# davidfang00/opticalflowdiffusion

Hardware: AMD Instinct MI355X
Metric: UNet denoise steps/sec @ 2x436x1024 flow, bs=16 (higher is better)
Workload: dtype bf16

## Files before the change

opticalflowdiffusion_amd/csrc/conv_common.h:

```cpp
#pragma once
#include "common.h"
#include "conv_params.h"
#include "mfma_util.h"

namespace ofd {

__device__ __forceinline__ float silu_f(float y) { return y * __builtin_amdgcn_rcpf(1.0f + __expf(-y)); }

static inline bool plain_epilogue(const ConvParams& P) {
    return !P.residual && !P.residual_b && !P.res_act && !P.split && !P.pool2 && !P.out2;
}

__device__ __forceinline__ u32x4 prologue_octet(u32x4 v, const float (&ps)[8], const float (&pb)[8]) {
#pragma unroll
    for (int j = 0; j < 4; ++j) {
        const float lo = silu_f(bf2f((bf16_t)(v[j] & 0xffffu)) * ps[2 * j] + pb[2 * j]);
        const float hi = silu_f(bf2f((bf16_t)(v[j] >> 16)) * ps[2 * j + 1] + pb[2 * j + 1]);
        v[j] = f2bf2(lo, hi);
    }
    return v;
}

__device__ __forceinline__ void load_in_affine8(const ConvParams& P, int b, int c_chunk, int c_oct, float (&ps)[8], float (&pb)[8]) {
    const float* sp = P.in_scale + (size_t)b * P.Cin_total + c_chunk + c_oct;
    const float* bp = P.in_shift + (size_t)b * P.Cin_total + c_chunk + c_oct;
    *(float4*)&ps[0] = *(const float4*)sp; *(float4*)&ps[4] = *(const float4*)(sp + 4);
    *(float4*)&pb[0] = *(const float4*)bp; *(float4*)&pb[4] = *(const float4*)(bp + 4);
}

__device__ __forceinline__ void split_quads(const uint4 t4, uint2& lo, uint2& hi) {
    const auto sx = __builtin_amdgcn_permlane32_swap(t4.x, t4.z, false, false);
    const auto sy = __builtin_amdgcn_permlane32_swap(t4.y, t4.w, false, false);
    lo = make_uint2(sx[0], sy[0]);
    hi = make_uint2(sx[1], sy[1]);
}

__device__ __forceinline__ void add_residual4(float (&v)[4], const uint2 t) {
    v[0] += bf2f((bf16_t)(t.x & 0xffffu));
    v[1] += bf2f((bf16_t)(t.x >> 16));
    v[2] += bf2f((bf16_t)(t.y & 0xffffu));
    v[3] += bf2f((bf16_t)(t.y >> 16));
}
__device__ __forceinline__ void add_silu_affine4(float (&v)[4], const uint2 t, const float4 sc, const float4 sh) {
    v[0] += silu_f(bf2f((bf16_t)(t.x & 0xffffu)) * sc.x + sh.x);
    v[1] += silu_f(bf2f((bf16_t)(t.x >> 16)) * sc.y + sh.y);
    v[2] += silu_f(bf2f((bf16_t)(t.y & 0xffffu)) * sc.z + sh.z);
    v[3] += silu_f(bf2f((bf16_t)(t.y >> 16)) * sc.w + sh.w);
}

__device__ __forceinline__ void gn_stat_add(const uint2 q, float& sum, float& sumsq) {
    typedef __bf16 bf16x2 __attribute__((ext_vector_type(2)));
    const bf16x2 one = __builtin_bit_cast(bf16x2, 0x3f803f80u);
    const bf16x2 va = __builtin_bit_cast(bf16x2, q.x), vb = __builtin_bit_cast(bf16x2, q.y);
    sum = __builtin_amdgcn_fdot2_f32_bf16(vb, one, __builtin_amdgcn_fdot2_f32_bf16(va, one, sum, false), false);
    sumsq = __builtin_amdgcn_fdot2_f32_bf16(vb, vb, __builtin_amdgcn_fdot2_f32_bf16(va, va, sumsq, false), false);
}

namespace wp {

constexpr int CK = 32, NC = CK / 8, IW = 34, TW = 32, RING = 6, FRAGS = 18;

template <int NS, int PH>
struct Cfg {
    static constexpr int NTHREADS = 64 * NS * PH;
    static constexpr int BN = 32 * NS, ROWS = 8 * PH, IH = ROWS + 2, NPIX = IH * IW;
    static constexpr int NC = wp::NC;
    static constexpr int US = (NPIX + 1) * 16;
    static constexpr int XB = NC * US;
    static constexpr int LDS_BYTES = 2 * XB;
    static constexpr int XPT = (NPIX * NC + NTHREADS - 1) / NTHREADS;
    static_assert(NS * PH == 4, "4 waves");
    static_assert((NPIX + 1) % 2 == 1, "odd slot count keeps the staging writes of a pixel's octets on distinct banks");
};

typedef u32x4 u4;

__device__ __forceinline__ bf16x8 as_frag(u4 v) { return __builtin_bit_cast(bf16x8, v); }

__device__ __forceinline__ void wave_reduce8(float (&v)[8]) {
    const int lane = threadIdx.x & 63;
#pragma unroll
    for (int i = 0; i < 4; ++i) {
        const auto r = __builtin_amdgcn_permlane32_swap(__float_as_uint(v[i]), __float_as_uint(v[i + 4]), false, false);
        v[i] = __uint_as_float(r[0]) + __uint_as_float(r[1]);
    }
#pragma unroll
    for (int i = 0; i < 2; ++i) {
        const auto r = __builtin_amdgcn_permlane16_swap(__float_as_uint(v[i]), __float_as_uint(v[i + 2]), false, false);
        v[i] = __uint_as_float(r[0]) + __uint_as_float(r[1]);
    }
    {
        const bool up = (lane & 8) != 0;
        const float send = up ? v[0] : v[1], keep = up ? v[1] : v[0];
        v[0] = keep + __uint_as_float(__builtin_amdgcn_mov_dpp(__float_as_uint(send), 0x128 , 0xf, 0xf, false));
    }
    v[0] += __uint_as_float(__builtin_amdgcn_mov_dpp(__float_as_uint(v[0]), 0x141 , 0xf, 0xf, false));
    v[0] += __uint_as_float(__builtin_amdgcn_mov_dpp(__float_as_uint(v[0]), 0xb1 , 0xf, 0xf, false));
    v[0] += __uint_as_float(__builtin_amdgcn_mov_dpp(__float_as_uint(v[0]), 0x4e , 0xf, 0xf, false));
}

template <int NS, int OCT>
__device__ __forceinline__ void gn_partial_store_wave(const ConvParams& P, float (&stat)[8], int b, int ty8, int tiles8, int tx, int ns, int oct0, int lane) {
    wave_reduce8(stat);
    if (ty8 < tiles8) {
        constexpr int PER_WAVE = (4 / NS) * OCT * 2;
        const int slot_i = lane / (OCT * 2), o = (lane % (OCT * 2)) >> 1, which = lane & 1;
        const float total = __shfl(stat[0], ((o & 3) * 2 + which) * 8, 64);
        if (lane < PER_WAVE) {
            const int slot = ns + slot_i * NS;
            const bool own = slot_i == 0 && (o >> 2) == ns;
            P.gn_partial[gn_partial_index(b, tiles8 * P.tiles_x * 4, (ty8 * P.tiles_x + tx) * 4 + slot, P.Cout / 8, oct0 + o) + which] = own ? total : 0.0f;
        }
    }
}

template <int BN>
__device__ __forceinline__ bool cy_fast_decode(const ConvParams& P, int ntiles, int& tile, int& cy) {
    tile = blockIdx.x;
    cy = blockIdx.y;
    if (P.cy_fast) {
        const int ny = P.Cout / BN, j = blockIdx.x, g = j >> 3;
        cy = g % ny;
        tile = (g / ny) * 8 + (j & 7);
        if (tile >= ntiles) return false;
    }
    return true;
}

template <class C>
__device__ __forceinline__ void stage_map(const ConvParams& P, int tid, int oy0, int ox0, int (&pyx)[C::XPT], unsigned& okmask) {
    okmask = 0;
#pragma unroll
    for (int i = 0; i < C::XPT; ++i) {
        const int p = min(tid / C::NC + i * (C::NTHREADS / C::NC), C::NPIX - 1);
        const int ty = p / IW, tx = p - ty * IW;
        const int iy = oy0 - 1 + ty, ix = ox0 - 1 + tx;
        const bool ok = iy >= 0 && iy < P.H && ix >= 0 && ix < P.W;
        okmask |= (ok ? 1u : 0u) << i;
        pyx[i] = (min(max(iy, 0), P.H - 1) << 16) | min(max(ix, 0), P.W - 1);
    }
}

template <class C, bool PRO>
__device__ __forceinline__ void stage_write(const u4 (&xs)[C::XPT], unsigned okmask, const float (&ps)[8], const float (&pb)[8], unsigned char* xbuf, int t) {
    const int c8 = t % C::NC;
#pragma unroll
    for (int i = 0; i < C::XPT; ++i) {
        const int p = min(t / C::NC + i * (C::NTHREADS / C::NC), C::NPIX - 1);
        u4 v = xs[i];
        if constexpr (PRO) v = prologue_octet(v, ps, pb);
        const bool ok = (okmask >> i) & 1u;
#pragma unroll
        for (int j = 0; j < 4; ++j) v[j] = ok ? v[j] : 0u;
        *(u4*)(xbuf + c8 * C::US + p * 16) = v;
    }
}

template <class C>
__device__ __forceinline__ void stage_write(const u4 (&xs)[C::XPT], unsigned okmask, unsigned char* xbuf, int t) {
    const float none[8] = {};
    stage_write<C, false>(xs, okmask, none, none, xbuf, t);
}

struct ChunkSrc {
    const bf16_t* base;
    int SW, stride;
    int up;
};
__device__ __forceinline__ ChunkSrc chunk_src(const ConvParams& P, int b, int kc, int c8, int& src_i, int& src_first) {
    const int k64 = kc >> 1;
    while (k64 >= src_first + P.src[src_i].chunks) {
        src_first += P.src[src_i].chunks;
        ++src_i;
    }
    const ConvSrcDev& S = P.src[src_i];
    return {S.ptr + (size_t)b * S.SH * S.SW * S.src_channels + S.ch_offset + (k64 - src_first) * 64 + (kc & 1) * CK + c8 * 8, S.SW, S.src_channels,
            S.mode == 1 ? 1 : 0};
}

template <class C>
__device__ __forceinline__ void load_chunk(const ConvParams& P, int b, int kc, int tid, const int (&pyx)[C::XPT], int& src_i, int& src_first, u4 (&xs)[C::XPT]) {
    const ChunkSrc S = chunk_src(P, b, kc, tid % C::NC, src_i, src_first);
#pragma unroll
    for (int i = 0; i < C::XPT; ++i) {
        const int sy = (pyx[i] >> 16) >> S.up, sx = (pyx[i] & 0xffff) >> S.up;
        xs[i] = *(const u4*)(S.base + ((size_t)sy * S.SW + sx) * S.stride);
    }
}
template <class C, bool PRO>
__device__ __forceinline__ void write_chunk(const ConvParams& P, int b, int kc, int tid, unsigned okmask, const u4 (&xs)[C::XPT], unsigned char* xbuf) {
    float ps[8], pb[8];
    if constexpr (PRO) load_in_affine8(P, b, kc * CK, (tid % C::NC) * 8, ps, pb);
    stage_write<C, PRO>(xs, okmask, ps, pb, xbuf, tid);
}

}

}
```

opticalflowdiffusion_amd/csrc/conv_pc.hip:

```cpp
#include <cstdlib>
#include <type_traits>
#include "conv_common.h"

namespace ofd {

namespace wp {

struct PcCfg {
    using C = Cfg<2, 2>;
    static constexpr int NPROD = C::NTHREADS, XPT = C::XPT;
    static constexpr int WSLOT = FRAGS * 2 * 1024;
    static constexpr int MAX_ITEMS = 512;
    static constexpr int ITEMS_OFF = 2 * C::XB + 2 * WSLOT;
    static constexpr int LDS_BYTES = ITEMS_OFF + MAX_ITEMS * 16;
};

template <bool PRO>
__global__ void __launch_bounds__(512, 2) conv3x3_pc_kernel(const ConvParams P) {
    using C = PcCfg::C;
    constexpr int NPROD = PcCfg::NPROD, XPT = PcCfg::XPT;
    extern __shared__ __attribute__((aligned(16))) unsigned char smem[];
    unsigned char* const wlds = smem + 2 * C::XB;
    const int tid = threadIdx.x;

    const int tiles_y = (P.H + C::ROWS - 1) / C::ROWS;
    const int tpi = P.tiles_x * tiles_y, ntiles = tpi * P.B, ny = P.Cout / C::BN, G = gridDim.x;
    const int nitems = (ntiles + 7) / 8 * 8 * ny;
    const int n32 = P.total_chunks * 2;
    auto decode = [&](int j, int& b, int& oy0, int& ox0, int& cy) -> bool {
        if (j >= nitems) return false;
        const int g = j >> 3;
        cy = ny > 1 ? g % ny : 0;
        int tile = (ny > 1 ? g / ny : g) * 8 + (j & 7);
        if (tile >= ntiles) return false;
        tile = xcd_tile_order(tile, ntiles);
        b = tile / tpi;
        const int t_in = tile - b * tpi;
        oy0 = (t_in / P.tiles_x) * C::ROWS;
        ox0 = (t_in % P.tiles_x) * TW;
        return true;
    };
    const int nit = blockIdx.x < nitems ? min((nitems - 1 - (int)blockIdx.x) / G + 1, PcCfg::MAX_ITEMS) : 0;
    int4* const items = (int4*)(smem + PcCfg::ITEMS_OFF);
    for (int k = tid; k < nit; k += 512) {
        int b_, y_, x_, c_;
        const bool ok = decode(blockIdx.x + k * G, b_, y_, x_, c_);
        items[k] = make_int4(ok ? b_ : -1, y_, x_, c_);
    }
    __syncthreads();
    int nvalid_items = 0;
    if (nit > 0) {
        int lo = 0, hi = nit;
        while (lo < hi) { const int mid = (lo + hi) >> 1; if (items[mid].x >= 0) lo = mid + 1; else hi = mid; }
        nvalid_items = lo;
    }
    const int T = n32 * nvalid_items;
    if (T == 0) return;
    auto item_at = [&](int k, int& b, int& oy0, int& ox0, int& cy) -> bool {
        if (k >= nvalid_items) return false;
        const int4 d = items[k];
        b = __builtin_amdgcn_readfirstlane(d.x); oy0 = __builtin_amdgcn_readfirstlane(d.y);
        ox0 = __builtin_amdgcn_readfirstlane(d.z); cy = __builtin_amdgcn_readfirstlane(d.w);
        return true;
    };

    if (tid >= 256) {
        const int ptid = tid - 256;
        const int c8 = ptid % NC;
        int tyx[XPT];
#pragma unroll
        for (int i = 0; i < XPT; ++i) {
            const int p = min(ptid / NC + i * (NPROD / NC), C::NPIX - 1);
            const int ty = p / IW;
            tyx[i] = (ty << 8) | (p - ty * IW);
        }
        int lk = 0, lkc = 0, lb, loy0, lox0, lcy;
        item_at(0, lb, loy0, lox0, lcy);
        auto advance = [&]() {
            if (++lkc == n32) {
                if (item_at(lk + 1, lb, loy0, lox0, lcy)) { lkc = 0; ++lk; }
                else lkc = n32 - 1;
            }
        };
        auto issue = [&](u4 (&xs)[XPT], unsigned& okmask, float (&ps)[8], float (&pb)[8]) {
            const int k64 = lkc >> 1;
            int si = 0, first = 0;
            while (k64 >= first + P.src[si].chunks) { first += P.src[si].chunks; ++si; }
            const ConvSrcDev& S = P.src[si];
            const bf16_t* base = S.ptr + (size_t)lb * S.SH * S.SW * S.src_channels + S.ch_offset + (k64 - first) * 64 + (lkc & 1) * CK + c8 * 8;
            const int up = S.mode == 1 ? 1 : 0;
            okmask = 0;
#pragma unroll
            for (int i = 0; i < XPT; ++i) {
                const int iy = loy0 - 1 + (tyx[i] >> 8), ix = lox0 - 1 + (tyx[i] & 0xff);
                const bool ok = iy >= 0 && iy < P.H && ix >= 0 && ix < P.W;
                okmask |= (ok ? 1u : 0u) << i;
                const int sy = min(max(iy, 0), P.H - 1) >> up, sx = min(max(ix, 0), P.W - 1) >> up;
                xs[i] = *(const u4*)(base + ((size_t)sy * S.SW + sx) * S.src_channels);
            }
            if constexpr (PRO) load_in_affine8(P, lb, lkc * CK, c8 * 8, ps, pb);
        };
        auto stage = [&](const u4 (&xs)[XPT], const unsigned okmask, const float (&ps)[8], const float (&pb)[8], unsigned char* xbuf) {
            stage_write<C, PRO>(xs, okmask, ps, pb, xbuf, ptid);
        };
        const int pw = __builtin_amdgcn_readfirstlane(ptid >> 6), plane_ = ptid & 63;
        const int cin8 = P.Cin_total / 8;
        const unsigned wlds_addr = (unsigned)(size_t)(__attribute__((address_space(3))) unsigned char*)wlds;
        int held0 = -1, held1 = -1;
        int sk = 0, skc = 0, scy, sb_, sy_, sx_;
        item_at(0, sb_, sy_, sx_, scy);
        auto stage_advance = [&]() {
            if (++skc == n32) {
                if (item_at(sk + 1, sb_, sy_, sx_, scy)) { skc = 0; ++sk; }
                else skc = n32 - 1;
            }
        };
        auto weights_dma = [&](const int slot) -> bool {
            const int key = (scy << 16) | skc;
            int& held = slot ? held1 : held0;
            if (held == key) return false;
            held = key;
#pragma unroll
            for (int q = 0; q < FRAGS * 2 / 4; ++q) {
                const int fr = pw * (FRAGS * 2 / 4) + q, fi = fr >> 1, ns_ = fr & 1;
                const int g = fi / 3, ky = fi - g * 3, ks = g / 3, kx = g - ks * 3;
                const int row = (ky * 3 + kx) * cin8 + skc * NC + ks * 2;
                const bf16_t* sbase = P.weight + ((size_t)row * P.Cout + scy * C::BN + 32 * ns_) * 8;
                const unsigned dst = wlds_addr + (unsigned)(((slot * FRAGS + fi) * 2 + ns_) * 1024);
                const unsigned voff = (unsigned)(((plane_ >> 5) * P.Cout + (plane_ & 31)) * 16);
                asm volatile("s_mov_b32 m0, %0\n\ts_nop 0\n\tglobal_load_lds_dwordx4 %1, %2" :: "s"(dst), "v"(voff), "s"(sbase) : "memory");
            }
            return true;
        };
        u4 x0[XPT], x1[XPT], x2[XPT];
        unsigned ok0 = 0, ok1 = 0, ok2 = 0;
        float ps0[8], pb0[8], ps1[8], pb1[8], ps2[8], pb2[8];
        weights_dma(0); stage_advance();
        issue(x0, ok0, ps0, pb0); advance();
        issue(x1, ok1, ps1, pb1); advance();
        issue(x2, ok2, ps2, pb2); advance();
        stage(x0, ok0, ps0, pb0, smem);
        asm volatile("s_waitcnt vmcnt(0)" ::: "memory");
        __syncthreads();
#define PC_STEP(XL, OKL, PSL, PBL, XS, OKS, PSS, PBS, BUF)                                          \
        {                                                                                           \
            if (i >= T) break;                                                                      \
            const bool wd_ = weights_dma(BUF);                  \
            stage_advance();                                                                        \
            issue(XL, OKL, PSL, PBL);                                                               \
            stage(XS, OKS, PSS, PBS, smem + (BUF) * C::XB);                                         \
            advance();                                                                              \
            if (wd_) asm volatile("s_waitcnt vmcnt(%0)" ::"n"(XPT + (PRO ? 4 : 0)) : "memory");     \
            __syncthreads();                                                                        \
            ++i;                                                                                    \
        }
        for (int i = 0; i < T;) {
            PC_STEP(x0, ok0, ps0, pb0, x1, ok1, ps1, pb1, 1)
            PC_STEP(x1, ok1, ps1, pb1, x2, ok2, ps2, pb2, 0)
            PC_STEP(x2, ok2, ps2, pb2, x0, ok0, ps0, pb0, 1)
            PC_STEP(x0, ok0, ps0, pb0, x1, ok1, ps1, pb1, 0)
            PC_STEP(x1, ok1, ps1, pb1, x2, ok2, ps2, pb2, 1)
            PC_STEP(x2, ok2, ps2, pb2, x0, ok0, ps0, pb0, 0)
        }
#undef PC_STEP
        return;
    }

    const int lane = tid & 63, wave = __builtin_amdgcn_readfirstlane(tid >> 6);
    const int l31 = lane & 31, half = lane >> 5;
    const int ns = wave & 1, ph = wave >> 1;
    __builtin_amdgcn_s_setprio(2);

    int ik = 0, b, oy0, ox0, cy;
    item_at(0, b, oy0, ox0, cy);

    f32x16 biasv;
    auto load_bias = [&](int cy_) {
#pragma unroll
        for (int g = 0; g < 4; ++g) {
            const float4 b4 = P.bias ? *(const float4*)(P.bias + cy_ * C::BN + 32 * ns + 8 * g + 4 * half) : make_float4(0.f, 0.f, 0.f, 0.f);
            biasv[4 * g] = b4.x; biasv[4 * g + 1] = b4.y; biasv[4 * g + 2] = b4.z; biasv[4 * g + 3] = b4.w;
        }
    };
    load_bias(cy);
    f32x16 acc[8];

    const int xrow_off = half * C::US + (8 * ph * IW + l31) * 16;
    const unsigned char* const wfrag = wlds + ns * 1024 + lane * 16;
    auto chunk = [&](const int slot, const unsigned char* xbase, auto first_tag) {
        constexpr bool FIRST = decltype(first_tag)::value;
        const unsigned char* xrow = xbase + xrow_off;
#pragma unroll
        for (int g = 0; g < 6; ++g) {
            const int ks = g / 3, kx = g % 3;
            bf16x8 x[10];
#pragma unroll
            for (int jr = 0; jr < 10; ++jr) x[jr] = *(const bf16x8*)(xrow + (jr * IW + kx) * 16 + ks * 2 * C::US);
            bf16x8 a[3];
#pragma unroll
            for (int ky = 0; ky < 3; ++ky) a[ky] = *(const bf16x8*)(wfrag + (slot * FRAGS + g * 3 + ky) * 2048);
#pragma unroll
            for (int r = 0; r < 8; ++r)
#pragma unroll
                for (int ky = 0; ky < 3; ++ky)
                    acc[r] = __builtin_amdgcn_mfma_f32_32x32x16_bf16(a[ky], x[r + ky], (FIRST && g == 0 && ky == 0) ? biasv : acc[r], 0, 0, 0);
        }
    };

    const int tiles8 = (P.H + 7) / 8;
    __syncthreads();
    while (true) {
        int nb, noy0, nox0, ncy;
        const bool nvalid = item_at(ik + 1, nb, noy0, nox0, ncy);
        for (int kc = 0; kc < n32; kc += 2) {
            if (kc == 0) chunk(0, smem, std::true_type{}); else chunk(0, smem, std::false_type{});
            __syncthreads();
            chunk(1, smem + C::XB, std::false_type{});
            __syncthreads();
        }
        __builtin_amdgcn_s_setprio(0);
        float stat[8];
#pragma unroll
        for (int i = 0; i < 8; ++i) stat[i] = 0.0f;
        const int oyb = oy0 + 8 * ph, ox = ox0 + l31, cb = cy * C::BN + 32 * ns;
        const bool okx = ox < P.W;
        const size_t oplane_b = (size_t)P.H * P.W * P.Cout * 2;
        const __amdgpu_buffer_rsrc_t orsrc = __builtin_amdgcn_make_buffer_rsrc((void*)(P.out + (size_t)b * P.H * P.W * P.Cout), 0, (int)oplane_b, 0x00020000);
        const unsigned olane = (unsigned)(((min(oyb, P.H - 1) * P.W + min(ox, P.W - 1)) * P.Cout + cb + 8 * half) * 2);
        const unsigned ostride_b = (unsigned)(P.W * P.Cout * 2);
        const bool full = ox0 + TW <= P.W && oyb + 8 <= P.H && oplane_b < (1ull << 31);
        if (full) {
#pragma unroll
            for (int r = 0; r < 8; ++r) {
                uint2 q[4];
#pragma unroll
                for (int g = 0; g < 4; ++g) {
                    q[g] = make_uint2(f2bf2(acc[r][4 * g], acc[r][4 * g + 1]), f2bf2(acc[r][4 * g + 2], acc[r][4 * g + 3]));
                    if (P.gn_partial) gn_stat_add(q[g], stat[g * 2], stat[g * 2 + 1]);
                }
#pragma unroll
                for (int g = 0; g < 4; g += 2) {
                    const auto rx = __builtin_amdgcn_permlane32_swap(q[g].x, q[g + 1].x, false, false);
                    const auto ry = __builtin_amdgcn_permlane32_swap(q[g].y, q[g + 1].y, false, false);
                    u4 pk = {rx[0], ry[0], rx[1], ry[1]};
                    __builtin_amdgcn_raw_buffer_store_b128(pk, orsrc, (int)olane, (int)(r * ostride_b + 16 * g), 0);
                }
            }
        } else {
        bf16_t* orow = P.out + (((size_t)b * P.H + min(oyb, P.H - 1)) * P.W + min(ox, P.W - 1)) * P.Cout + cb + 8 * half;
        const size_t ostride = (size_t)P.W * P.Cout;
#pragma unroll
        for (int r = 0; r < 8; ++r) {
            const bool ok = okx && oyb + r < P.H;
            uint2 q[4];
#pragma unroll
            for (int g = 0; g < 4; ++g) {
                q[g] = make_uint2(f2bf2(acc[r][4 * g], acc[r][4 * g + 1]), f2bf2(acc[r][4 * g + 2], acc[r][4 * g + 3]));
                if (P.gn_partial && ok) gn_stat_add(q[g], stat[g * 2], stat[g * 2 + 1]);
            }
#pragma unroll
            for (int g = 0; g < 4; g += 2) {
                const auto rx = __builtin_amdgcn_permlane32_swap(q[g].x, q[g + 1].x, false, false);
                const auto ry = __builtin_amdgcn_permlane32_swap(q[g].y, q[g + 1].y, false, false);
                if (ok) *(uint4*)(orow + 8 * g) = make_uint4(rx[0], ry[0], rx[1], ry[1]);
            }
            orow += ostride;
        }
        }
        if (P.gn_partial) gn_partial_store_wave<2, C::BN / 8>(P, stat, b, oy0 / 8 + ph, tiles8, ox0 / TW, ns, cy * C::BN / 8, lane);
        if (!nvalid) break;
        ++ik; b = nb; oy0 = noy0; ox0 = nox0;
        if (ncy != cy) { cy = ncy; load_bias(cy); }
        __builtin_amdgcn_s_setprio(2);
    }
}

static bool pc_serves(const ConvParams& P) {
    for (int i = 0; i < P.n_src; ++i)
        if (P.src[i].mode != 0 && P.src[i].mode != 1) return false;
    return P.Cout % 64 == 0 && plain_epilogue(P) && P.W <= 8160 ;
}

}

int launch_conv3x3_pc(const ConvParams& P, hipStream_t s) {
    using namespace wp;
    using C = PcCfg::C;
    if (!pc_serves(P)) return 1;
    static int cus = 0;
    if (!cus) {
        int dev = 0, n = 0;
        OFD_HIP(hipGetDevice(&dev));
        OFD_HIP(hipDeviceGetAttribute(&n, hipDeviceAttributeMultiprocessorCount, dev));
        OFD_HIP(hipFuncSetAttribute((const void*)conv3x3_pc_kernel<false>, hipFuncAttributeMaxDynamicSharedMemorySize, PcCfg::LDS_BYTES));
        OFD_HIP(hipFuncSetAttribute((const void*)conv3x3_pc_kernel<true>, hipFuncAttributeMaxDynamicSharedMemorySize, PcCfg::LDS_BYTES));
        cus = n / 8 * 8 < 8 ? 8 : n / 8 * 8;
    }
    const int tiles_y = (P.H + C::ROWS - 1) / C::ROWS;
    const int ntiles = P.tiles_x * tiles_y * P.B, ny = P.Cout / C::BN;
    const int nitems = (ntiles + 7) / 8 * 8 * ny;
    const int grid = nitems < cus ? nitems : cus;
    if ((long)grid * PcCfg::MAX_ITEMS < nitems) return 1;
    if (P.in_scale) conv3x3_pc_kernel<true><<<grid, 512, PcCfg::LDS_BYTES, s>>>(P);
    else conv3x3_pc_kernel<false><<<grid, 512, PcCfg::LDS_BYTES, s>>>(P);
    OFD_LAUNCH_CHECK();
    return OFD_OK;
}

}
```

opticalflowdiffusion_amd/csrc/conv_wp.hip:

```cpp
#include <cstdlib>
#include <type_traits>
#include "conv_common.h"

namespace ofd {

namespace wp {

template <int NS, int PH, bool PRO>
__global__ void __launch_bounds__(64 * NS * PH, 2) conv3x3_wp_kernel(const ConvParams P) {
    using C = Cfg<NS, PH>;
    extern __shared__ __attribute__((aligned(16))) unsigned char smem[];

    const int tid = threadIdx.x, lane = tid & 63, wave = tid >> 6;
    const int l31 = lane & 31, half = lane >> 5;
    const int ns = wave % NS, ph = wave / NS;

    const int tiles_y = (P.H + C::ROWS - 1) / C::ROWS;
    const int tpi = P.tiles_x * tiles_y, ntiles = tpi * P.B;
    int tile, cy;
    if (!cy_fast_decode<C::BN>(P, ntiles, tile, cy)) return;
    tile = xcd_tile_order(tile, ntiles);
    const int b = tile / tpi, t_in = tile % tpi;
    const int oy0 = (t_in / P.tiles_x) * C::ROWS, ox0 = (t_in % P.tiles_x) * TW;
    const int n0 = cy * C::BN;
    const int cb = n0 + 32 * ns;

    const int cin8 = P.Cin_total / 8, n32 = P.total_chunks * 2;
    const __amdgpu_buffer_rsrc_t wrsrc = __builtin_amdgcn_make_buffer_rsrc((void*)P.weight, 0, 9 * P.Cin_total * P.Cout * 2, 0x00020000);
    const int w_lane = (half * P.Cout + cb + l31) * 16;
    const int w_row = P.Cout * 16;
    auto load_w = [&](int kc, int fi) -> u4 {
        const int g = fi / 3, ky = fi % 3, ks = g / 3, kx = g % 3;
        const int row = (ky * 3 + kx) * cin8 + kc * NC + ks * 2;
        return __builtin_bit_cast(u4, __builtin_amdgcn_raw_buffer_load_b128(wrsrc, w_lane, row * w_row, 0));
    };
    u4 ring[RING];
#pragma unroll
    for (int i = 0; i < RING; ++i) ring[i] = load_w(0, i);

    int pyx[C::XPT];
    unsigned okmask;
    stage_map<C>(P, tid, oy0, ox0, pyx, okmask);
    int src_i = 0, src_first = 0;
    auto load_x = [&](int kc, u4 (&xs)[C::XPT]) { load_chunk<C>(P, b, kc, tid, pyx, src_i, src_first, xs); };
    auto write_x = [&](int kc, const u4 (&xs)[C::XPT], unsigned char* xbuf) { write_chunk<C, PRO>(P, b, kc, tid, okmask, xs, xbuf); };

    f32x16 acc[8];
#pragma unroll
    for (int r = 0; r < 8; ++r)
#pragma unroll
        for (int k = 0; k < 16; ++k) acc[r][k] = 0.0f;

    u4 xs[C::XPT];
    load_x(0, xs);
    write_x(0, xs, smem);

    const int xrow_off = half * C::US + (8 * ph * IW + l31) * 16;
    auto chunk = [&](const int kc, auto last_tag) {
        constexpr bool LAST = decltype(last_tag)::value;
        const int kn = LAST ? kc : kc + 1;
        if constexpr (!LAST) load_x(kn, xs);
        __syncthreads();
        const unsigned char* xrow = smem + (kc & 1) * C::XB + xrow_off;
        unsigned char* xnext = smem + ((kc + 1) & 1) * C::XB;
#pragma unroll
        for (int g = 0; g < 6; ++g) {
            const int ks = g / 3, kx = g % 3;
            bf16x8 x[10];
#pragma unroll
            for (int j = 0; j < 10; ++j) x[j] = *(const bf16x8*)(xrow + (j * IW + kx) * 16 + ks * 2 * C::US);
            bf16x8 a[3];
#pragma unroll
            for (int ky = 0; ky < 3; ++ky) {
                const int fi = g * 3 + ky;
                a[ky] = as_frag(ring[fi % RING]);
                if (fi + RING < FRAGS) ring[fi % RING] = load_w(kc, fi + RING);
                else if constexpr (!LAST) ring[fi % RING] = load_w(kn, fi + RING - FRAGS);
            }
#pragma unroll
            for (int r = 0; r < 8; ++r)
#pragma unroll
                for (int ky = 0; ky < 3; ++ky) acc[r] = __builtin_amdgcn_mfma_f32_32x32x16_bf16(a[ky], x[r + ky], acc[r], 0, 0, 0);
            if constexpr (!LAST) { if (g == 1) write_x(kn, xs, xnext); }
        }
    };
    for (int kc = 0; kc < n32 - 1; ++kc) chunk(kc, std::false_type{});
    chunk(n32 - 1, std::true_type{});

    float stat[8];
#pragma unroll
    for (int i = 0; i < 8; ++i) stat[i] = 0.0f;
    const bool second = P.split > 0 && cb >= P.split;
    bf16_t* const o_base = second ? P.out2 : P.out;
    const bf16_t* const r_base = second ? P.residual2 : P.residual;
    const int o_stride = P.split > 0 ? (second ? P.Cout - P.split : P.split) : P.Cout;
    const int o_c0 = cb - (second ? P.split : 0);
    float4 bias4[4];
#pragma unroll
    for (int g = 0; g < 4; ++g) bias4[g] = P.bias ? *(const float4*)(P.bias + cb + 8 * g + 4 * half) : make_float4(0.f, 0.f, 0.f, 0.f);
    if (P.pool2) {
        const int PH2 = P.H >> 1, PW2 = P.W >> 1;
#pragma unroll
        for (int i = 0; i < 4; ++i) {
            const int py = ((oy0 + 8 * ph) >> 1) + i, px = (ox0 + l31) >> 1;
            const bool ok = py < PH2 && px < PW2 && !(l31 & 1);
            const size_t pix = ((size_t)b * PH2 + min(py, PH2 - 1)) * PW2 + min(px, PW2 - 1);
            uint2 q[4], rr[4];
            if (r_base) {
#pragma unroll
                for (int g = 0; g < 4; g += 2) split_quads(*(const uint4*)(r_base + pix * o_stride + o_c0 + 8 * g + 8 * half), rr[g], rr[g + 1]);
            }
#pragma unroll
            for (int g = 0; g < 4; ++g) {
                float v[4];
#pragma unroll
                for (int k = 0; k < 4; ++k) {
                    v[k] = acc[2 * i][4 * g + k] + acc[2 * i + 1][4 * g + k];
                    v[k] += __shfl_xor(v[k], 1, 64);
                }
                v[0] += 4.0f * bias4[g].x; v[1] += 4.0f * bias4[g].y; v[2] += 4.0f * bias4[g].z; v[3] += 4.0f * bias4[g].w;
                if (r_base) add_residual4(v, rr[g]);
                q[g] = make_uint2(f2bf2(v[0], v[1]), f2bf2(v[2], v[3]));
            }
#pragma unroll
            for (int g = 0; g < 4; g += 2) {
                const auto rx = __builtin_amdgcn_permlane32_swap(q[g].x, q[g + 1].x, false, false);
                const auto ry = __builtin_amdgcn_permlane32_swap(q[g].y, q[g + 1].y, false, false);
                if (ok) *(uint4*)(o_base + pix * o_stride + o_c0 + 8 * g + 8 * half) = make_uint4(rx[0], ry[0], rx[1], ry[1]);
            }
        }
        return;
    }
#pragma unroll
    for (int r = 0; r < 8; ++r) {
        const int oy = oy0 + 8 * ph + r, ox = ox0 + l31;
        const bool ok = oy < P.H && ox < P.W;
        const size_t pix = ((size_t)b * P.H + min(oy, P.H - 1)) * P.W + min(ox, P.W - 1);
        uint2 q[4], ra[4], rr[4];
        if (P.residual_b) {
#pragma unroll
            for (int g = 0; g < 4; g += 2) {
                uint2 rb[2];
                split_quads(*(const uint4*)(P.residual_b + pix * o_stride + o_c0 + 8 * g + 8 * half), rb[0], rb[1]);
#pragma unroll
                for (int h = 0; h < 2; ++h) {
                    float v[4] = {acc[r][4 * (g + h)], acc[r][4 * (g + h) + 1], acc[r][4 * (g + h) + 2], acc[r][4 * (g + h) + 3]};
                    add_residual4(v, rb[h]);
#pragma unroll
                    for (int k = 0; k < 4; ++k) acc[r][4 * (g + h) + k] = v[k];
                }
            }
        }
        if (P.res_act) {
#pragma unroll
            for (int g = 0; g < 4; g += 2) split_quads(*(const uint4*)(P.res_act + pix * P.Cout + cb + 8 * g + 8 * half), ra[g], ra[g + 1]);
        }
        if (r_base) {
#pragma unroll
            for (int g = 0; g < 4; g += 2) split_quads(*(const uint4*)(r_base + pix * o_stride + o_c0 + 8 * g + 8 * half), rr[g], rr[g + 1]);
        }
#pragma unroll
        for (int g = 0; g < 4; ++g) {
            const int c = cb + 8 * g + 4 * half;
            float v[4] = {acc[r][4 * g] + bias4[g].x, acc[r][4 * g + 1] + bias4[g].y, acc[r][4 * g + 2] + bias4[g].z, acc[r][4 * g + 3] + bias4[g].w};
            if (P.res_act)
                add_silu_affine4(v, ra[g], *(const float4*)(P.res_scale + (size_t)b * P.Cout + c), *(const float4*)(P.res_shift + (size_t)b * P.Cout + c));
            if (r_base) add_residual4(v, rr[g]);
            q[g] = make_uint2(f2bf2(v[0], v[1]), f2bf2(v[2], v[3]));
            if (P.gn_partial && ok) gn_stat_add(q[g], stat[g * 2], stat[g * 2 + 1]);
        }
#pragma unroll
        for (int g = 0; g < 4; g += 2) {
            const auto rx = __builtin_amdgcn_permlane32_swap(q[g].x, q[g + 1].x, false, false);
            const auto ry = __builtin_amdgcn_permlane32_swap(q[g].y, q[g + 1].y, false, false);
            if (ok) *(uint4*)(o_base + pix * o_stride + o_c0 + 8 * g + 8 * half) = make_uint4(rx[0], ry[0], rx[1], ry[1]);
        }
    }

    if (P.gn_partial) gn_partial_store_wave<NS, C::BN / 8>(P, stat, b, oy0 / 8 + ph, (P.H + 7) / 8, t_in % P.tiles_x, ns, n0 / 8, lane);
}

typedef __attribute__((ext_vector_type(4))) float f32x4;

template <bool PRO>
__global__ void __launch_bounds__(256, 2) conv3x3_wp16_kernel(const ConvParams P) {
    using C = Cfg<4, 1>;
    extern __shared__ __attribute__((aligned(16))) unsigned char smem[];
    const int tid = threadIdx.x, lane = tid & 63, ns = tid >> 6;
    const int l15 = lane & 15, lg = lane >> 4;

    const int tiles_y = (P.H + C::ROWS - 1) / C::ROWS;
    const int tpi = P.tiles_x * tiles_y, ntiles = tpi * P.B;
    int tile, cy;
    if (!cy_fast_decode<C::BN>(P, ntiles, tile, cy)) return;
    tile = xcd_tile_order(tile, ntiles);
    const int b = tile / tpi, t_in = tile % tpi;
    const int oy0 = (t_in / P.tiles_x) * C::ROWS, ox0 = (t_in % P.tiles_x) * TW;
    const int cb = cy * C::BN + 32 * ns;

    const int cin8 = P.Cin_total / 8, n32 = P.total_chunks * 2;
    const __amdgpu_buffer_rsrc_t wrsrc = __builtin_amdgcn_make_buffer_rsrc((void*)P.weight, 0, 9 * P.Cin_total * P.Cout * 2, 0x00020000);
    const int w_lane = (lg * P.Cout + cb + l15) * 16;
    const int w_row = P.Cout * 16;
    auto load_w = [&](int kc, int kx, int i) -> u4 {
        const int ky = i >> 1, h = i & 1;
        const int row = (ky * 3 + kx) * cin8 + kc * NC;
        return __builtin_bit_cast(u4, __builtin_amdgcn_raw_buffer_load_b128(wrsrc, w_lane + h * 256, row * w_row, 0));
    };

    int pyx[C::XPT];
    unsigned okmask;
    stage_map<C>(P, tid, oy0, ox0, pyx, okmask);
    int src_i = 0, src_first = 0;
    auto load_x = [&](int kc, u4 (&xs)[C::XPT]) { load_chunk<C>(P, b, kc, tid, pyx, src_i, src_first, xs); };
    auto write_x = [&](int kc, const u4 (&xs)[C::XPT], unsigned char* xbuf) { write_chunk<C, PRO>(P, b, kc, tid, okmask, xs, xbuf); };

    f32x4 acc[8][2][2];
#pragma unroll
    for (int r = 0; r < 8; ++r)
#pragma unroll
        for (int q = 0; q < 4; ++q)
#pragma unroll
            for (int k = 0; k < 4; ++k) acc[r][q >> 1][q & 1][k] = 0.0f;

    u4 xs[C::XPT];
    load_x(0, xs);
    write_x(0, xs, smem);
    u4 wa[6], wb[6];
#pragma unroll
    for (int i = 0; i < 6; ++i) wa[i] = load_w(0, 0, i);

    const int xrow_off = lg * C::US + l15 * 16;
    auto column = [&](const unsigned char* xrow, const int kx, u4 (&cur)[6], u4 (&nxt)[6], const int nkc, const int nkx, const bool fetch) {
        if (fetch) {
#pragma unroll
            for (int i = 0; i < 6; ++i) nxt[i] = load_w(nkc, nkx, i);
        }
#pragma unroll
        for (int p = 0; p < 2; ++p)
#pragma unroll
            for (int hf = 0; hf < 2; ++hf) {
                bf16x8 x[6];
#pragma unroll
                for (int j = 0; j < 6; ++j) x[j] = *(const bf16x8*)(xrow + ((4 * hf + j) * IW + kx + 16 * p) * 16);
#pragma unroll
                for (int r = 0; r < 4; ++r)
#pragma unroll
                    for (int ky = 0; ky < 3; ++ky)
#pragma unroll
                        for (int h = 0; h < 2; ++h)
                            acc[4 * hf + r][p][h] = __builtin_amdgcn_mfma_f32_16x16x32_bf16(as_frag(cur[ky * 2 + h]), x[r + ky], acc[4 * hf + r][p][h], 0, 0, 0);
            }
    };
    auto chunk = [&](const int kc, auto even_tag, auto last_tag) {
        constexpr bool EVEN = decltype(even_tag)::value, LAST = decltype(last_tag)::value;
        const int kn = LAST ? kc : kc + 1;
        if constexpr (!LAST) load_x(kn, xs);
        __syncthreads();
        const unsigned char* xrow = smem + (kc & 1) * C::XB + xrow_off;
        unsigned char* xnext = smem + ((kc + 1) & 1) * C::XB;
        if constexpr (EVEN) {
            column(xrow, 0, wa, wb, kc, 1, true);
            if constexpr (!LAST) write_x(kn, xs, xnext);
            column(xrow, 1, wb, wa, kc, 2, true);
            column(xrow, 2, wa, wb, kn, 0, !LAST);
        } else {
            column(xrow, 0, wb, wa, kc, 1, true);
            if constexpr (!LAST) write_x(kn, xs, xnext);
            column(xrow, 1, wa, wb, kc, 2, true);
            column(xrow, 2, wb, wa, kn, 0, !LAST);
        }
    };
    for (int kc = 0; kc < n32 - 2; kc += 2) {
        chunk(kc, std::true_type{}, std::false_type{});
        chunk(kc + 1, std::false_type{}, std::false_type{});
    }
    chunk(n32 - 2, std::true_type{}, std::false_type{});
    chunk(n32 - 1, std::false_type{}, std::true_type{});

    float4 bias4[2];
#pragma unroll
    for (int h = 0; h < 2; ++h) bias4[h] = P.bias ? *(const float4*)(P.bias + cb + 16 * h + 4 * lg) : make_float4(0.f, 0.f, 0.f, 0.f);
    float st[2][2] = {{0.0f, 0.0f}, {0.0f, 0.0f}};
    const int c_store = cb + 16 * (lg & 1) + 8 * (lg >> 1);
#pragma unroll
    for (int r = 0; r < 8; ++r) {
        const int oy = oy0 + r;
#pragma unroll
        for (int p = 0; p < 2; ++p) {
            const int ox = ox0 + 16 * p + l15;
            const bool ok = oy < P.H && ox < P.W;
            const size_t pix = ((size_t)b * P.H + min(oy, P.H - 1)) * P.W + min(ox, P.W - 1);
            uint2 q[2];
#pragma unroll
            for (int h = 0; h < 2; ++h) {
                const f32x4 a = acc[r][p][h];
                q[h] = make_uint2(f2bf2(a[0] + bias4[h].x, a[1] + bias4[h].y), f2bf2(a[2] + bias4[h].z, a[3] + bias4[h].w));
                if (P.gn_partial && ok) gn_stat_add(q[h], st[h][0], st[h][1]);
            }
            const auto rx = __builtin_amdgcn_permlane16_swap(q[0].x, q[1].x, false, false);
            const auto ry = __builtin_amdgcn_permlane16_swap(q[0].y, q[1].y, false, false);
            if (ok) *(uint4*)(P.out + pix * P.Cout + c_store) = make_uint4(rx[0], ry[0], rx[1], ry[1]);
        }
    }
    if (P.gn_partial) {
#pragma unroll
        for (int h = 0; h < 2; ++h)
#pragma unroll
            for (int w = 0; w < 2; ++w) {
                float v = st[h][w];
                v += __shfl_xor(v, 1, 64); v += __shfl_xor(v, 2, 64); v += __shfl_xor(v, 4, 64); v += __shfl_xor(v, 8, 64); v += __shfl_xor(v, 16, 64);
                st[h][w] = v;
            }
        const int ty8 = oy0 / 8, tiles8 = (P.H + 7) / 8;
        if (ty8 < tiles8) {
            constexpr int OCT = C::BN / 8, PER_WAVE = OCT * 2;
            const int o = (lane % PER_WAVE) >> 1, which = lane & 1;
            const int oo = o & 3, hh = oo >> 1, mm = oo & 1;
            const float t00 = __shfl(st[0][0], mm * 32, 64), t01 = __shfl(st[0][1], mm * 32, 64);
            const float t10 = __shfl(st[1][0], mm * 32, 64), t11 = __shfl(st[1][1], mm * 32, 64);
            const float total = hh ? (which ? t11 : t10) : (which ? t01 : t00);
            if (lane < PER_WAVE) {
                const bool own = (o >> 2) == ns;
                P.gn_partial[gn_partial_index(b, tiles8 * P.tiles_x * 4, (ty8 * P.tiles_x + (t_in % P.tiles_x)) * 4 + ns, P.Cout / 8, cy * C::BN / 8 + o) + which] =
                    own ? total : 0.0f;
            }
        }
    }
}

static int wp_lds_attributes() {
    static bool done = false;
    if (!done) {
        OFD_HIP(hipFuncSetAttribute((const void*)conv3x3_wp_kernel<4, 1, false>, hipFuncAttributeMaxDynamicSharedMemorySize, Cfg<4, 1>::LDS_BYTES));
        OFD_HIP(hipFuncSetAttribute((const void*)conv3x3_wp_kernel<4, 1, true>, hipFuncAttributeMaxDynamicSharedMemorySize, Cfg<4, 1>::LDS_BYTES));
        OFD_HIP(hipFuncSetAttribute((const void*)conv3x3_wp_kernel<2, 2, false>, hipFuncAttributeMaxDynamicSharedMemorySize, Cfg<2, 2>::LDS_BYTES));
        OFD_HIP(hipFuncSetAttribute((const void*)conv3x3_wp_kernel<2, 2, true>, hipFuncAttributeMaxDynamicSharedMemorySize, Cfg<2, 2>::LDS_BYTES));
        OFD_HIP(hipFuncSetAttribute((const void*)conv3x3_wp16_kernel<false>, hipFuncAttributeMaxDynamicSharedMemorySize, Cfg<4, 1>::LDS_BYTES));
        OFD_HIP(hipFuncSetAttribute((const void*)conv3x3_wp16_kernel<true>, hipFuncAttributeMaxDynamicSharedMemorySize, Cfg<4, 1>::LDS_BYTES));
        done = true;
    }
    return OFD_OK;
}

template <class C>
static int launch(void (*kernel)(const ConvParams), const ConvParams& P, hipStream_t s) {
    const int rc = wp_lds_attributes();
    if (rc) return rc;
    const int tiles_y = (P.H + C::ROWS - 1) / C::ROWS;
    const int ntiles = P.tiles_x * tiles_y * P.B, ny = P.Cout / C::BN;
    dim3 grid(ntiles, ny);
    if (P.cy_fast) grid = dim3((ntiles + 7) / 8 * 8 * ny, 1);
    kernel<<<grid, C::NTHREADS, C::LDS_BYTES, s>>>(P);
    OFD_LAUNCH_CHECK();
    return OFD_OK;
}

}

int launch_conv3x3_pc(const ConvParams& P, hipStream_t s);

int launch_conv3x3_wp(const ConvParams& P0, bool wide, hipStream_t s) {
    ConvParams P = P0;
    P.cy_fast = P.Cout / (wide ? 128 : 64) > 1;
    using W = wp::Cfg<4, 1>;
    using N = wp::Cfg<2, 2>;
    if (wide && plain_epilogue(P)) return P.in_scale ? wp::launch<W>(wp::conv3x3_wp16_kernel<true>, P, s) : wp::launch<W>(wp::conv3x3_wp16_kernel<false>, P, s);
    if (!wide && env_int("OFD_CONV_PC", 1)) {
        const int r = launch_conv3x3_pc(P, s);
        if (r != 1) return r;
    }
    if (P.in_scale) return wide ? wp::launch<W>(wp::conv3x3_wp_kernel<4, 1, true>, P, s) : wp::launch<N>(wp::conv3x3_wp_kernel<2, 2, true>, P, s);
    return wide ? wp::launch<W>(wp::conv3x3_wp_kernel<4, 1, false>, P, s) : wp::launch<N>(wp::conv3x3_wp_kernel<2, 2, false>, P, s);
}

}
```

Before: 34.40.

## Overlap conv epilogue stores with next tile's MFMA in producer-consumer kernel

```diff
diff --git a/opticalflowdiffusion_amd/csrc/conv_common.h b/opticalflowdiffusion_amd/csrc/conv_common.h
--- a/opticalflowdiffusion_amd/csrc/conv_common.h
+++ b/opticalflowdiffusion_amd/csrc/conv_common.h
@@ -100,8 +100,7 @@
 }
 
 template <int NS, int OCT>
-__device__ __forceinline__ void gn_partial_store_wave(const ConvParams& P, float (&stat)[8], int b, int ty8, int tiles8, int tx, int ns, int oct0, int lane) {
-    wave_reduce8(stat);
+__device__ __forceinline__ void gn_partial_store_reduced(const ConvParams& P, const float (&stat)[8], int b, int ty8, int tiles8, int tx, int ns, int oct0, int lane) {
     if (ty8 < tiles8) {
         constexpr int PER_WAVE = (4 / NS) * OCT * 2;
         const int slot_i = lane / (OCT * 2), o = (lane % (OCT * 2)) >> 1, which = lane & 1;
@@ -112,6 +111,12 @@
             P.gn_partial[gn_partial_index(b, tiles8 * P.tiles_x * 4, (ty8 * P.tiles_x + tx) * 4 + slot, P.Cout / 8, oct0 + o) + which] = own ? total : 0.0f;
         }
     }
+}
+
+template <int NS, int OCT>
+__device__ __forceinline__ void gn_partial_store_wave(const ConvParams& P, float (&stat)[8], int b, int ty8, int tiles8, int tx, int ns, int oct0, int lane) {
+    wave_reduce8(stat);
+    gn_partial_store_reduced<NS, OCT>(P, stat, b, ty8, tiles8, tx, ns, oct0, lane);
 }
 
 template <int BN>
diff --git a/opticalflowdiffusion_amd/csrc/conv_pc.hip b/opticalflowdiffusion_amd/csrc/conv_pc.hip
--- a/opticalflowdiffusion_amd/csrc/conv_pc.hip
+++ b/opticalflowdiffusion_amd/csrc/conv_pc.hip
@@ -14,6 +14,15 @@
     static constexpr int ITEMS_OFF = 2 * C::XB + 2 * WSLOT;
     static constexpr int LDS_BYTES = ITEMS_OFF + MAX_ITEMS * 16;
 };
+
+template <int NM, int NV>
+__device__ __forceinline__ void mfma_valu_interleave() {
+#pragma unroll
+    for (int i = 0; i < NM; ++i) {
+        __builtin_amdgcn_sched_group_barrier(0x008, 1, 0);
+        __builtin_amdgcn_sched_group_barrier(0x002, NV, 0);
+    }
+}
 
 template <bool PRO>
 __global__ void __launch_bounds__(512, 2) conv3x3_pc_kernel(const ConvParams P) {
@@ -64,7 +73,7 @@
         return true;
     };
 
-    if (tid >= 256) {
+    if (__builtin_amdgcn_readfirstlane(tid >> 8)) {
         const int ptid = tid - 256;
         const int c8 = ptid % NC;
         int tyx[XPT];
@@ -206,9 +215,156 @@
                     acc[r] = __builtin_amdgcn_mfma_f32_32x32x16_bf16(a[ky], x[r + ky], (FIRST && g == 0 && ky == 0) ? biasv : acc[r], 0, 0, 0);
         }
     };
+    auto half_chunk = [&](const int slot, const unsigned char* xbase, auto first_tag, auto rh_tag) {
+        constexpr bool FIRST = decltype(first_tag)::value;
+        constexpr int R0 = 4 * decltype(rh_tag)::value;
+        const unsigned char* xrow = xbase + xrow_off + R0 * IW * 16;
+#pragma unroll
+        for (int g = 0; g < 6; ++g) {
+            const int ks = g / 3, kx = g % 3;
+            bf16x8 x[6];
+#pragma unroll
+            for (int jr = 0; jr < 6; ++jr) x[jr] = *(const bf16x8*)(xrow + (jr * IW + kx) * 16 + ks * 2 * C::US);
+            bf16x8 a[3];
+#pragma unroll
+            for (int ky = 0; ky < 3; ++ky) a[ky] = *(const bf16x8*)(wfrag + (slot * FRAGS + g * 3 + ky) * 2048);
+#pragma unroll
+            for (int r = 0; r < 4; ++r)
+#pragma unroll
+                for (int ky = 0; ky < 3; ++ky)
+                    acc[R0 + r] = __builtin_amdgcn_mfma_f32_32x32x16_bf16(a[ky], x[r + ky], (FIRST && g == 0 && ky == 0) ? biasv : acc[R0 + r], 0, 0, 0);
+        }
+    };
 
     const int tiles8 = (P.H + 7) / 8;
+    const size_t oplane_b = (size_t)P.H * P.W * P.Cout * 2;
+    const unsigned ostride_b = (unsigned)(P.W * P.Cout * 2);
+    const int full_x = oplane_b < (1ull << 31) ? P.W - TW : -1, full_y = P.H - 8 * ph - 8;
+    auto tile_full = [&](int oy0_, int ox0_) -> bool { return ox0_ <= full_x && oy0_ <= full_y; };
+    auto epilogue_full = [&](auto rh_tag, auto gn_tag, const bool en, int b_, int oy0_, int ox0_, int cy_, float (&stat)[8]) {
+        constexpr int R0 = 4 * decltype(rh_tag)::value;
+        constexpr bool GN = decltype(gn_tag)::value;
+        const int oyb = oy0_ + 8 * ph, ox = ox0_ + l31, cb = cy_ * C::BN + 32 * ns;
+        const __amdgpu_buffer_rsrc_t orsrc = __builtin_amdgcn_make_buffer_rsrc((void*)((unsigned char*)P.out + b_ * oplane_b), 0, en ? (int)oplane_b : 0, 0x00020000);
+        const unsigned olane = (unsigned)(((oyb * P.W + ox) * P.Cout + cb + 8 * half) * 2) | (en ? 0u : 0x80000000u);
+#pragma unroll
+        for (int r = R0; r < R0 + 4; ++r) {
+            uint2 q[4];
+#pragma unroll
+            for (int g = 0; g < 4; ++g) {
+                q[g] = make_uint2(f2bf2(acc[r][4 * g], acc[r][4 * g + 1]), f2bf2(acc[r][4 * g + 2], acc[r][4 * g + 3]));
+                if constexpr (GN) gn_stat_add(q[g], stat[g * 2], stat[g * 2 + 1]);
+            }
+#pragma unroll
+            for (int g = 0; g < 4; g += 2) {
+                const auto rx = __builtin_amdgcn_permlane32_swap(q[g].x, q[g + 1].x, false, false);
+                const auto ry = __builtin_amdgcn_permlane32_swap(q[g].y, q[g + 1].y, false, false);
+                u4 pk = {rx[0], ry[0], rx[1], ry[1]};
+                __builtin_amdgcn_raw_buffer_store_b128(pk, orsrc, (int)olane, (int)(r * ostride_b + 16 * g), 0);
+            }
+        }
+    };
+    auto epilogue_edge = [&](auto rh_tag, auto gn_tag, int b_, int oy0_, int ox0_, int cy_, float (&stat)[8]) {
+        constexpr int R0 = 4 * decltype(rh_tag)::value;
+        constexpr bool GN = decltype(gn_tag)::value;
+        const int oyb = oy0_ + 8 * ph, ox = ox0_ + l31, cb = cy_ * C::BN + 32 * ns;
+        const bool okx = ox < P.W;
+        const size_t ostride = (size_t)P.W * P.Cout;
+        bf16_t* orow = (bf16_t*)((unsigned char*)P.out + b_ * oplane_b) + ((size_t)min(oyb, P.H - 1) * P.W + min(ox, P.W - 1)) * P.Cout + cb + 8 * half + R0 * ostride;
+#pragma unroll
+        for (int r = R0; r < R0 + 4; ++r) {
+            const bool ok = okx && oyb + r < P.H;
+            uint2 q[4];
+#pragma unroll
+            for (int g = 0; g < 4; ++g) {
+                q[g] = make_uint2(f2bf2(acc[r][4 * g], acc[r][4 * g + 1]), f2bf2(acc[r][4 * g + 2], acc[r][4 * g + 3]));
+                if (GN && ok) gn_stat_add(q[g], stat[g * 2], stat[g * 2 + 1]);
+            }
+#pragma unroll
+            for (int g = 0; g < 4; g += 2) {
+                const auto rx = __builtin_amdgcn_permlane32_swap(q[g].x, q[g + 1].x, false, false);
+                const auto ry = __builtin_amdgcn_permlane32_swap(q[g].y, q[g + 1].y, false, false);
+                if (ok) *(uint4*)(orow + 8 * g) = make_uint4(rx[0], ry[0], rx[1], ry[1]);
+            }
+            orow += ostride;
+        }
+    };
+    constexpr std::integral_constant<int, 0> HA{};
+    constexpr std::integral_constant<int, 1> HB{};
+    auto walk = [&](auto gn_tag) {
+        constexpr bool GN = decltype(gn_tag)::value;
+        float stat[8], st[8];
+#pragma unroll
+        for (int i = 0; i < 8; ++i) stat[i] = 0.0f;
+#pragma unroll
+        for (int r = 4; r < 8; ++r) acc[r] = biasv;
+        while (true) {
+            const bool pending = ik > 0;
+            {
+                int pb = b, poy0 = oy0, pox0 = ox0, pcy = cy;
+                if (pending) item_at(ik - 1, pb, poy0, pox0, pcy);
+                const bool en = pending && tile_full(poy0, pox0);
+                __builtin_amdgcn_sched_barrier(0);
+                half_chunk(0, smem, std::true_type{}, HA);
+#pragma unroll
+                for (int i = 0; i < 8; ++i) st[i] = stat[i];
+                epilogue_full(HB, gn_tag, en, pb, poy0, pox0, pcy, st);
+                if constexpr (GN) wave_reduce8(st);
+                mfma_valu_interleave<72, 3>();
+                __builtin_amdgcn_sched_barrier(0);
+                if (pending) {
+                    if (en) {
+                        if constexpr (GN) gn_partial_store_reduced<2, C::BN / 8>(P, st, pb, poy0 / 8 + ph, tiles8, pox0 / TW, ns, pcy * C::BN / 8, lane);
+                    } else {
+                        __builtin_amdgcn_s_setprio(0);
+                        epilogue_edge(HB, gn_tag, pb, poy0, pox0, pcy, stat);
+                        if constexpr (GN) gn_partial_store_wave<2, C::BN / 8>(P, stat, pb, poy0 / 8 + ph, tiles8, pox0 / TW, ns, pcy * C::BN / 8, lane);
+                        __builtin_amdgcn_s_setprio(2);
+                    }
+                }
+            }
+            half_chunk(0, smem, std::true_type{}, HB);
+            __syncthreads();
+            for (int kc = 1; kc < n32 - 1; kc += 2) {
+                chunk(1, smem + C::XB, std::false_type{});
+                __syncthreads();
+                chunk(0, smem, std::false_type{});
+                __syncthreads();
+            }
+            half_chunk(1, smem + C::XB, std::false_type{}, HA);
+            {
+                const bool en = tile_full(oy0, ox0);
+                __builtin_amdgcn_sched_barrier(0);
+                half_chunk(1, smem + C::XB, std::false_type{}, HB);
+#pragma unroll
+                for (int i = 0; i < 8; ++i) stat[i] = 0.0f;
+                epilogue_full(HA, gn_tag, en, b, oy0, ox0, cy, stat);
+                mfma_valu_interleave<72, 3>();
+                __builtin_amdgcn_sched_barrier(0);
+                if (!en) {
+#pragma unroll
+                    for (int i = 0; i < 8; ++i) stat[i] = 0.0f;
+                    __builtin_amdgcn_s_setprio(0);
+                    epilogue_edge(HA, gn_tag, b, oy0, ox0, cy, stat);
+                    __builtin_amdgcn_s_setprio(2);
+                }
+            }
+            __syncthreads();
+            if (ik + 1 >= nvalid_items) break;
+            const int cy_was = cy;
+            item_at(++ik, b, oy0, ox0, cy);
+            if (cy != cy_was) load_bias(cy);
+        }
+        __builtin_amdgcn_s_setprio(0);
+        if (tile_full(oy0, ox0)) epilogue_full(HB, gn_tag, true, b, oy0, ox0, cy, stat);
+        else epilogue_edge(HB, gn_tag, b, oy0, ox0, cy, stat);
+        if constexpr (GN) gn_partial_store_wave<2, C::BN / 8>(P, stat, b, oy0 / 8 + ph, tiles8, ox0 / TW, ns, cy * C::BN / 8, lane);
+    };
     __syncthreads();
+    if constexpr (PRO) {
+        if (P.gn_partial) walk(std::true_type{}); else walk(std::false_type{});
+        return;
+    }
     while (true) {
         int nb, noy0, nox0, ncy;
         const bool nvalid = item_at(ik + 1, nb, noy0, nox0, ncy);
```

Result: no change. 34.72 (median of 6 runs) (+0.9%).

## Interleave weight and activation loads between MFMA slots in wp16 conv kernel

Applied to the files above, without the earlier changes.

```diff
diff --git a/opticalflowdiffusion_amd/csrc/conv_wp.hip b/opticalflowdiffusion_amd/csrc/conv_wp.hip
--- a/opticalflowdiffusion_amd/csrc/conv_wp.hip
+++ b/opticalflowdiffusion_amd/csrc/conv_wp.hip
@@ -212,7 +212,15 @@
     unsigned okmask;
     stage_map<C>(P, tid, oy0, ox0, pyx, okmask);
     int src_i = 0, src_first = 0;
-    auto load_x = [&](int kc, u4 (&xs)[C::XPT]) { load_chunk<C>(P, b, kc, tid, pyx, src_i, src_first, xs); };
+    const unsigned oct_off = (tid % C::NC) * 16;
+    auto src_of = [&](int kc) { return chunk_src(P, b, kc, 0, src_i, src_first); };
+    auto load_x = [&](const ChunkSrc& S, u4 (&xs)[C::XPT]) {
+#pragma unroll
+        for (int i = 0; i < C::XPT; ++i) {
+            const unsigned sy = (unsigned)pyx[i] >> (16 + S.up), sx = __builtin_amdgcn_ubfe((unsigned)pyx[i], S.up, 16 - S.up);
+            xs[i] = *(const u4*)((const unsigned char*)S.base + ((sy * S.SW + sx) * (S.stride * 2) + oct_off));
+        }
+    };
     auto write_x = [&](int kc, const u4 (&xs)[C::XPT], unsigned char* xbuf) { write_chunk<C, PRO>(P, b, kc, tid, okmask, xs, xbuf); };
 
     f32x4 acc[8][2][2];
@@ -224,22 +232,19 @@
             for (int k = 0; k < 4; ++k) acc[r][q >> 1][q & 1][k] = 0.0f;
 
     u4 xs[C::XPT];
-    load_x(0, xs);
+    load_x(src_of(0), xs);
     write_x(0, xs, smem);
     u4 wa[6], wb[6];
 #pragma unroll
     for (int i = 0; i < 6; ++i) wa[i] = load_w(0, 0, i);
 
     const int xrow_off = lg * C::US + l15 * 16;
-    auto column = [&](const unsigned char* xrow, const int kx, u4 (&cur)[6], u4 (&nxt)[6], const int nkc, const int nkx, const bool fetch) {
-        if (fetch) {
-#pragma unroll
-            for (int i = 0; i < 6; ++i) nxt[i] = load_w(nkc, nkx, i);
-        }
+    auto mfma_column = [&](const unsigned char* xrow, const int kx, const u4 (&cur)[6], auto before) {
 #pragma unroll
         for (int p = 0; p < 2; ++p)
 #pragma unroll
             for (int hf = 0; hf < 2; ++hf) {
+                before(kx * 4 + p * 2 + hf);
                 bf16x8 x[6];
 #pragma unroll
                 for (int j = 0; j < 6; ++j) x[j] = *(const bf16x8*)(xrow + ((4 * hf + j) * IW + kx + 16 * p) * 16);
@@ -252,24 +257,40 @@
                             acc[4 * hf + r][p][h] = __builtin_amdgcn_mfma_f32_16x16x32_bf16(as_frag(cur[ky * 2 + h]), x[r + ky], acc[4 * hf + r][p][h], 0, 0, 0);
             }
     };
+    auto fetch_w = [&](u4 (&nxt)[6], const int kc, const int kx) {
+#pragma unroll
+        for (int i = 0; i < 6; ++i) nxt[i] = load_w(kc, kx, i);
+    };
     auto chunk = [&](const int kc, auto even_tag, auto last_tag) {
         constexpr bool EVEN = decltype(even_tag)::value, LAST = decltype(last_tag)::value;
+        constexpr int FENCE = 0x386;
         const int kn = LAST ? kc : kc + 1;
-        if constexpr (!LAST) load_x(kn, xs);
+        ChunkSrc S = {};
+        if constexpr (!LAST) S = src_of(kn);
         __syncthreads();
         const unsigned char* xrow = smem + (kc & 1) * C::XB + xrow_off;
         unsigned char* xnext = smem + ((kc + 1) & 1) * C::XB;
-        if constexpr (EVEN) {
-            column(xrow, 0, wa, wb, kc, 1, true);
-            if constexpr (!LAST) write_x(kn, xs, xnext);
-            column(xrow, 1, wb, wa, kc, 2, true);
-            column(xrow, 2, wa, wb, kn, 0, !LAST);
-        } else {
-            column(xrow, 0, wb, wa, kc, 1, true);
-            if constexpr (!LAST) write_x(kn, xs, xnext);
-            column(xrow, 1, wa, wb, kc, 2, true);
-            column(xrow, 2, wb, wa, kn, 0, !LAST);
-        }
+        auto body = [&](u4 (&s0)[6], u4 (&s1)[6]) {
+            auto before = [&](const int slot) {
+                if (slot != 2 && slot != 6 && (LAST || (slot != 8 && slot != 10))) return;
+                __builtin_amdgcn_sched_barrier(FENCE);
+                if (slot == 2) fetch_w(s1, kc, 1);
+                if (slot == 6) fetch_w(s0, kc, 2);
+                if constexpr (!LAST) {
+                    if (slot == 8) load_x(S, xs);
+                    if (slot == 10) fetch_w(s1, kn, 0);
+                }
+                __builtin_amdgcn_sched_barrier(FENCE);
+            };
+            mfma_column(xrow, 0, s0, before);
+            mfma_column(xrow, 1, s1, before);
+            mfma_column(xrow, 2, s0, before);
+            if constexpr (!LAST) {
+                if constexpr (!PRO) __builtin_amdgcn_sched_barrier(0x384);
+                write_x(kn, xs, xnext);
+            }
+        };
+        if constexpr (EVEN) body(wa, wb); else body(wb, wa);
     };
     for (int kc = 0; kc < n32 - 2; kc += 2) {
         chunk(kc, std::true_type{}, std::false_type{});
@@ -365,7 +386,9 @@
     P.cy_fast = P.Cout / (wide ? 128 : 64) > 1;
     using W = wp::Cfg<4, 1>;
     using N = wp::Cfg<2, 2>;
-    if (wide && plain_epilogue(P)) return P.in_scale ? wp::launch<W>(wp::conv3x3_wp16_kernel<true>, P, s) : wp::launch<W>(wp::conv3x3_wp16_kernel<false>, P, s);
+    bool off32 = true;
+    for (int i = 0; i < P.n_src; ++i) off32 = off32 && (size_t)P.src[i].SH * P.src[i].SW * P.src[i].src_channels * 2 < ((size_t)1 << 32);
+    if (wide && off32 && plain_epilogue(P)) return P.in_scale ? wp::launch<W>(wp::conv3x3_wp16_kernel<true>, P, s) : wp::launch<W>(wp::conv3x3_wp16_kernel<false>, P, s);
     if (!wide && env_int("OFD_CONV_PC", 1)) {
         const int r = launch_conv3x3_pc(P, s);
         if (r != 1) return r;
```

Measured after the change: 34.54 before, 35.10 after, median of 6. +1.6%, better.
